# PaddlePaddle/PaddleNLP

Measured on NVIDIA H100. Metric: tokens/sec Llama-3.2-3B seq4096 bf16 pretrain step (global, all GPUs), higher is better.
Workload: dtype bf16

## Files before the change

### paddlenlp_b200/csrc/common.cuh

```cuda
#pragma once
#include <cuda.h>
#include <cuda_bf16.h>
#include <cuda_runtime.h>
#include <stdint.h>
#include <stdio.h>

namespace b200 {

typedef __nv_bfloat16 bf16;

__device__ __forceinline__ uint32_t smem_u32(const void* p) {
  return static_cast<uint32_t>(__cvta_generic_to_shared(p));
}
__device__ __forceinline__ void named_bar_sync(uint32_t id, uint32_t nthreads) {
  asm volatile("bar.sync %0, %1;" ::"r"(id), "r"(nthreads) : "memory");
}

__device__ __forceinline__ void pdl_wait() { asm volatile("griddepcontrol.wait;" ::: "memory"); }
__device__ __forceinline__ void pdl_launch_dependents() { asm volatile("griddepcontrol.launch_dependents;" ::: "memory"); }

__device__ __forceinline__ void mbar_init(uint64_t* bar, uint32_t count) {
  asm volatile("mbarrier.init.shared::cta.b64 [%0], %1;" ::"r"(smem_u32(bar)), "r"(count) : "memory");
}
__device__ __forceinline__ void fence_mbar_init() {
  asm volatile("fence.mbarrier_init.release.cluster;" ::: "memory");
}
__device__ __forceinline__ void fence_proxy_async_smem() {
  asm volatile("fence.proxy.async.shared::cta;" ::: "memory");
}
__device__ __forceinline__ void mbar_arrive_expect_tx(uint64_t* bar, uint32_t bytes) {
  asm volatile("mbarrier.arrive.expect_tx.shared::cta.b64 _, [%0], %1;" ::"r"(smem_u32(bar)), "r"(bytes)
               : "memory");
}
__device__ __forceinline__ void mbar_arrive(uint64_t* bar) {
  asm volatile("mbarrier.arrive.shared::cta.b64 _, [%0];" ::"r"(smem_u32(bar)) : "memory");
}
__device__ __forceinline__ bool mbar_try_wait(uint64_t* bar, uint32_t parity) {
  uint32_t ok;
  asm volatile(
      "{\n\t.reg .pred P;\n\t"
      "mbarrier.try_wait.parity.shared::cta.b64 P, [%1], %2;\n\t"
      "selp.u32 %0, 1, 0, P;\n\t}\n"
      : "=r"(ok)
      : "r"(smem_u32(bar)), "r"(parity)
      : "memory");
  return ok != 0;
}
__device__ __forceinline__ void mbar_wait(uint64_t* bar, uint32_t parity) {
  if (mbar_try_wait(bar, parity)) return;
  long long t0 = clock64();
  uint32_t spins = 0;
  while (!mbar_try_wait(bar, parity)) {
    if ((++spins & 0x3FFu) == 0 && (clock64() - t0) > 8000000000LL) {
      printf("[b200 watchdog] mbarrier wait timed out: block %d thread %d bar 0x%x parity %u\n", (int)blockIdx.x,
             (int)threadIdx.x, smem_u32(bar), parity);
      __trap();
    }
  }
}
__device__ __forceinline__ void mbar_wait_nocall(uint64_t* bar, uint32_t parity) {
  if (mbar_try_wait(bar, parity)) return;
  long long t0 = clock64();
  uint32_t spins = 0;
  while (!mbar_try_wait(bar, parity)) {
    if ((++spins & 0x3FFu) == 0 && (clock64() - t0) > 8000000000LL) __trap();
  }
}

__device__ __forceinline__ void tma_prefetch_desc(const CUtensorMap* tm) {
  asm volatile("prefetch.tensormap [%0];" ::"l"(reinterpret_cast<uint64_t>(tm)) : "memory");
}
__device__ __forceinline__ void tma_load_2d(const CUtensorMap* tm, uint64_t* bar, void* smem_dst, int c0, int c1) {
  asm volatile(
      "cp.async.bulk.tensor.2d.shared::cluster.global.mbarrier::complete_tx::bytes [%0], [%1, {%3, %4}], [%2];"
      ::"r"(smem_u32(smem_dst)), "l"(reinterpret_cast<uint64_t>(tm)), "r"(smem_u32(bar)), "r"(c0), "r"(c1)
      : "memory");
}
__device__ __forceinline__ void bulk_load(void* smem_dst, const void* src, uint32_t bytes, uint64_t* bar) {
  asm volatile("cp.async.bulk.shared::cluster.global.mbarrier::complete_tx::bytes [%0], [%1], %2, [%3];" ::"r"(smem_u32(smem_dst)),
               "l"(src), "r"(bytes), "r"(smem_u32(bar))
               : "memory");
}
__device__ __forceinline__ void tma_load_4d(const CUtensorMap* tm, uint64_t* bar, void* smem_dst, int c0, int c1,
                                            int c2, int c3) {
  asm volatile(
      "cp.async.bulk.tensor.4d.shared::cluster.global.mbarrier::complete_tx::bytes [%0], [%1, {%3, %4, %5, %6}], [%2];"
      ::"r"(smem_u32(smem_dst)), "l"(reinterpret_cast<uint64_t>(tm)), "r"(smem_u32(bar)), "r"(c0), "r"(c1), "r"(c2),
      "r"(c3)
      : "memory");
}
__device__ __forceinline__ void tma_reduce_add_4d(const CUtensorMap* tm, const void* smem_src, int c0, int c1, int c2,
                                                  int c3) {
  asm volatile("cp.reduce.async.bulk.tensor.4d.global.shared::cta.add.tile.bulk_group [%0, {%2, %3, %4, %5}], [%1];" ::"l"(
                   reinterpret_cast<uint64_t>(tm)),
               "r"(smem_u32(smem_src)), "r"(c0), "r"(c1), "r"(c2), "r"(c3)
               : "memory");
}
__device__ __forceinline__ void tma_store_commit() { asm volatile("cp.async.bulk.commit_group;" ::: "memory"); }
template <int N>
__device__ __forceinline__ void tma_store_wait_read() {
  asm volatile("cp.async.bulk.wait_group.read %0;" ::"n"(N) : "memory");
}
template <int N>
__device__ __forceinline__ void tma_store_wait() {
  asm volatile("cp.async.bulk.wait_group %0;" ::"n"(N) : "memory");
}

__device__ __forceinline__ uint64_t wgmma_desc_sw128(uint32_t saddr, uint32_t lbo_bytes, uint32_t sbo_bytes) {
  uint64_t d = 0;
  d |= static_cast<uint64_t>((saddr & 0x3FFFFu) >> 4);
  d |= static_cast<uint64_t>((lbo_bytes >> 4) & 0x3FFFu) << 16;
  d |= static_cast<uint64_t>((sbo_bytes >> 4) & 0x3FFFu) << 32;
  d |= static_cast<uint64_t>(1) << 62;
  return d;
}
__device__ __forceinline__ void wgmma_fence() { asm volatile("wgmma.fence.sync.aligned;" ::: "memory"); }
__device__ __forceinline__ void wgmma_commit() { asm volatile("wgmma.commit_group.sync.aligned;" ::: "memory"); }
template <int N>
__device__ __forceinline__ void wgmma_wait() { asm volatile("wgmma.wait_group.sync.aligned %0;" ::"n"(N) : "memory"); }
template <int R>
__device__ __forceinline__ void setmaxnreg_dec() { asm volatile("setmaxnreg.dec.sync.aligned.u32 %0;" ::"n"(R)); }
template <int R>
__device__ __forceinline__ void setmaxnreg_inc() { asm volatile("setmaxnreg.inc.sync.aligned.u32 %0;" ::"n"(R)); }

template <int TA, int TB>
__device__ __forceinline__ void wgmma_m64n256k16(float (&d)[128], uint64_t desc_a, uint64_t desc_b, uint32_t accumulate) {
  asm volatile(
      "{\n\t.reg .pred p;\n\tsetp.ne.b32 p, %130, 0;\n\t"
      "wgmma.mma_async.sync.aligned.m64n256k16.f32.bf16.bf16 "
      "{%0, %1, %2, %3, %4, %5, %6, %7, %8, %9, %10, %11, %12, %13, %14, %15, %16, %17, %18, %19, %20, %21, %22, %23, %24, %25, %26, %27, %28, %29, %30, %31, %32, %33, %34, %35, %36, %37, %38, %39, %40, %41, %42, %43, %44, %45, %46, %47, %48, %49, %50, %51, %52, %53, %54, %55, %56, %57, %58, %59, %60, %61, %62, %63, %64, %65, %66, %67, %68, %69, %70, %71, %72, %73, %74, %75, %76, %77, %78, %79, %80, %81, %82, %83, %84, %85, %86, %87, %88, %89, %90, %91, %92, %93, %94, %95, %96, %97, %98, %99, %100, %101, %102, %103, %104, %105, %106, %107, %108, %109, %110, %111, %112, %113, %114, %115, %116, %117, %118, %119, %120, %121, %122, %123, %124, %125, %126, %127}, %128, %129, p, 1, 1, %131, %132;\n\t}\n"
      : "+f"(d[0]), "+f"(d[1]), "+f"(d[2]), "+f"(d[3]), "+f"(d[4]), "+f"(d[5]), "+f"(d[6]), "+f"(d[7]), "+f"(d[8]), "+f"(d[9]), "+f"(d[10]), "+f"(d[11]), "+f"(d[12]), "+f"(d[13]), "+f"(d[14]), "+f"(d[15]), "+f"(d[16]), "+f"(d[17]), "+f"(d[18]), "+f"(d[19]), "+f"(d[20]), "+f"(d[21]), "+f"(d[22]), "+f"(d[23]), "+f"(d[24]), "+f"(d[25]), "+f"(d[26]), "+f"(d[27]), "+f"(d[28]), "+f"(d[29]), "+f"(d[30]), "+f"(d[31]), "+f"(d[32]), "+f"(d[33]), "+f"(d[34]), "+f"(d[35]), "+f"(d[36]), "+f"(d[37]), "+f"(d[38]), "+f"(d[39]), "+f"(d[40]), "+f"(d[41]), "+f"(d[42]), "+f"(d[43]), "+f"(d[44]), "+f"(d[45]), "+f"(d[46]), "+f"(d[47]), "+f"(d[48]), "+f"(d[49]), "+f"(d[50]), "+f"(d[51]), "+f"(d[52]), "+f"(d[53]), "+f"(d[54]), "+f"(d[55]), "+f"(d[56]), "+f"(d[57]), "+f"(d[58]), "+f"(d[59]), "+f"(d[60]), "+f"(d[61]), "+f"(d[62]), "+f"(d[63]), "+f"(d[64]), "+f"(d[65]), "+f"(d[66]), "+f"(d[67]), "+f"(d[68]), "+f"(d[69]), "+f"(d[70]), "+f"(d[71]), "+f"(d[72]), "+f"(d[73]), "+f"(d[74]), "+f"(d[75]), "+f"(d[76]), "+f"(d[77]), "+f"(d[78]), "+f"(d[79]), "+f"(d[80]), "+f"(d[81]), "+f"(d[82]), "+f"(d[83]), "+f"(d[84]), "+f"(d[85]), "+f"(d[86]), "+f"(d[87]), "+f"(d[88]), "+f"(d[89]), "+f"(d[90]), "+f"(d[91]), "+f"(d[92]), "+f"(d[93]), "+f"(d[94]), "+f"(d[95]), "+f"(d[96]), "+f"(d[97]), "+f"(d[98]), "+f"(d[99]), "+f"(d[100]), "+f"(d[101]), "+f"(d[102]), "+f"(d[103]), "+f"(d[104]), "+f"(d[105]), "+f"(d[106]), "+f"(d[107]), "+f"(d[108]), "+f"(d[109]), "+f"(d[110]), "+f"(d[111]), "+f"(d[112]), "+f"(d[113]), "+f"(d[114]), "+f"(d[115]), "+f"(d[116]), "+f"(d[117]), "+f"(d[118]), "+f"(d[119]), "+f"(d[120]), "+f"(d[121]), "+f"(d[122]), "+f"(d[123]), "+f"(d[124]), "+f"(d[125]), "+f"(d[126]), "+f"(d[127])
      : "l"(desc_a), "l"(desc_b), "r"(accumulate), "n"(TA), "n"(TB));
}
template <int TA, int TB>
__device__ __forceinline__ void wgmma_m64n64k16(float (&d)[32], uint64_t desc_a, uint64_t desc_b, uint32_t accumulate) {
  asm volatile(
      "{\n\t.reg .pred p;\n\tsetp.ne.b32 p, %34, 0;\n\t"
      "wgmma.mma_async.sync.aligned.m64n64k16.f32.bf16.bf16 "
      "{%0, %1, %2, %3, %4, %5, %6, %7, %8, %9, %10, %11, %12, %13, %14, %15, %16, %17, %18, %19, %20, %21, %22, %23, %24, %25, %26, %27, %28, %29, %30, %31}, %32, %33, p, 1, 1, %35, %36;\n\t}\n"
      : "+f"(d[0]), "+f"(d[1]), "+f"(d[2]), "+f"(d[3]), "+f"(d[4]), "+f"(d[5]), "+f"(d[6]), "+f"(d[7]), "+f"(d[8]), "+f"(d[9]), "+f"(d[10]), "+f"(d[11]), "+f"(d[12]), "+f"(d[13]), "+f"(d[14]), "+f"(d[15]), "+f"(d[16]), "+f"(d[17]), "+f"(d[18]), "+f"(d[19]), "+f"(d[20]), "+f"(d[21]), "+f"(d[22]), "+f"(d[23]), "+f"(d[24]), "+f"(d[25]), "+f"(d[26]), "+f"(d[27]), "+f"(d[28]), "+f"(d[29]), "+f"(d[30]), "+f"(d[31])
      : "l"(desc_a), "l"(desc_b), "r"(accumulate), "n"(TA), "n"(TB));
}
template <int TB>
__device__ __forceinline__ void wgmma_m64n128k16_rs(float (&d)[64], const uint32_t* a, uint64_t desc_b, uint32_t accumulate) {
  asm volatile(
      "{\n\t.reg .pred p;\n\tsetp.ne.b32 p, %69, 0;\n\t"
      "wgmma.mma_async.sync.aligned.m64n128k16.f32.bf16.bf16 "
      "{%0, %1, %2, %3, %4, %5, %6, %7, %8, %9, %10, %11, %12, %13, %14, %15, %16, %17, %18, %19, %20, %21, %22, %23, %24, %25, %26, %27, %28, %29, %30, %31, %32, %33, %34, %35, %36, %37, %38, %39, %40, %41, %42, %43, %44, %45, %46, %47, %48, %49, %50, %51, %52, %53, %54, %55, %56, %57, %58, %59, %60, %61, %62, %63}, {%64, %65, %66, %67}, %68, p, 1, 1, %70;\n\t}\n"
      : "+f"(d[0]), "+f"(d[1]), "+f"(d[2]), "+f"(d[3]), "+f"(d[4]), "+f"(d[5]), "+f"(d[6]), "+f"(d[7]), "+f"(d[8]), "+f"(d[9]), "+f"(d[10]), "+f"(d[11]), "+f"(d[12]), "+f"(d[13]), "+f"(d[14]), "+f"(d[15]), "+f"(d[16]), "+f"(d[17]), "+f"(d[18]), "+f"(d[19]), "+f"(d[20]), "+f"(d[21]), "+f"(d[22]), "+f"(d[23]), "+f"(d[24]), "+f"(d[25]), "+f"(d[26]), "+f"(d[27]), "+f"(d[28]), "+f"(d[29]), "+f"(d[30]), "+f"(d[31]), "+f"(d[32]), "+f"(d[33]), "+f"(d[34]), "+f"(d[35]), "+f"(d[36]), "+f"(d[37]), "+f"(d[38]), "+f"(d[39]), "+f"(d[40]), "+f"(d[41]), "+f"(d[42]), "+f"(d[43]), "+f"(d[44]), "+f"(d[45]), "+f"(d[46]), "+f"(d[47]), "+f"(d[48]), "+f"(d[49]), "+f"(d[50]), "+f"(d[51]), "+f"(d[52]), "+f"(d[53]), "+f"(d[54]), "+f"(d[55]), "+f"(d[56]), "+f"(d[57]), "+f"(d[58]), "+f"(d[59]), "+f"(d[60]), "+f"(d[61]), "+f"(d[62]), "+f"(d[63])
      : "r"(a[0]), "r"(a[1]), "r"(a[2]), "r"(a[3]), "l"(desc_b), "r"(accumulate), "n"(TB));
}
template <int TB>
__device__ __forceinline__ void wgmma_m64n64k16_rs(float (&d)[32], const uint32_t* a, uint64_t desc_b, uint32_t accumulate) {
  asm volatile(
      "{\n\t.reg .pred p;\n\tsetp.ne.b32 p, %37, 0;\n\t"
      "wgmma.mma_async.sync.aligned.m64n64k16.f32.bf16.bf16 "
      "{%0, %1, %2, %3, %4, %5, %6, %7, %8, %9, %10, %11, %12, %13, %14, %15, %16, %17, %18, %19, %20, %21, %22, %23, %24, %25, %26, %27, %28, %29, %30, %31}, {%32, %33, %34, %35}, %36, p, 1, 1, %38;\n\t}\n"
      : "+f"(d[0]), "+f"(d[1]), "+f"(d[2]), "+f"(d[3]), "+f"(d[4]), "+f"(d[5]), "+f"(d[6]), "+f"(d[7]), "+f"(d[8]), "+f"(d[9]), "+f"(d[10]), "+f"(d[11]), "+f"(d[12]), "+f"(d[13]), "+f"(d[14]), "+f"(d[15]), "+f"(d[16]), "+f"(d[17]), "+f"(d[18]), "+f"(d[19]), "+f"(d[20]), "+f"(d[21]), "+f"(d[22]), "+f"(d[23]), "+f"(d[24]), "+f"(d[25]), "+f"(d[26]), "+f"(d[27]), "+f"(d[28]), "+f"(d[29]), "+f"(d[30]), "+f"(d[31])
      : "r"(a[0]), "r"(a[1]), "r"(a[2]), "r"(a[3]), "l"(desc_b), "r"(accumulate), "n"(TB));
}

__device__ __forceinline__ void mma_bf16_16816(float (&c)[4], const uint32_t (&a)[4], uint32_t b0, uint32_t b1) {
  asm volatile(
      "mma.sync.aligned.m16n8k16.row.col.f32.bf16.bf16.f32 {%0, %1, %2, %3}, {%4, %5, %6, %7}, {%8, %9}, "
      "{%0, %1, %2, %3};"
      : "+f"(c[0]), "+f"(c[1]), "+f"(c[2]), "+f"(c[3])
      : "r"(a[0]), "r"(a[1]), "r"(a[2]), "r"(a[3]), "r"(b0), "r"(b1));
}
__device__ __forceinline__ void ldsm_x4(uint32_t saddr, uint32_t (&r)[4]) {
  asm volatile("ldmatrix.sync.aligned.m8n8.x4.shared.b16 {%0, %1, %2, %3}, [%4];"
               : "=r"(r[0]), "=r"(r[1]), "=r"(r[2]), "=r"(r[3])
               : "r"(saddr));
}
__device__ __forceinline__ void ldsm_x4_t(uint32_t saddr, uint32_t (&r)[4]) {
  asm volatile("ldmatrix.sync.aligned.m8n8.x4.trans.shared.b16 {%0, %1, %2, %3}, [%4];"
               : "=r"(r[0]), "=r"(r[1]), "=r"(r[2]), "=r"(r[3])
               : "r"(saddr));
}
__device__ __forceinline__ void cp_async_16(uint32_t saddr, const void* gptr, uint32_t src_bytes) {
  asm volatile("cp.async.cg.shared.global [%0], [%1], 16, %2;" ::"r"(saddr), "l"(gptr), "r"(src_bytes) : "memory");
}
__device__ __forceinline__ void cp_async_commit() { asm volatile("cp.async.commit_group;" ::: "memory"); }
template <int N>
__device__ __forceinline__ void cp_async_wait() { asm volatile("cp.async.wait_group %0;" ::"n"(N) : "memory"); }

__device__ __forceinline__ uint32_t pack_bf16x2(float lo, float hi) {
  __nv_bfloat162 v = __floats2bfloat162_rn(lo, hi);
  return *reinterpret_cast<uint32_t*>(&v);
}
__device__ __forceinline__ float2 unpack_bf16x2(uint32_t u) {
  __nv_bfloat162 v = *reinterpret_cast<__nv_bfloat162*>(&u);
  return __bfloat1622float2(v);
}
__device__ __forceinline__ float bf16_round(float x) { return __bfloat162float(__float2bfloat16_rn(x)); }

__device__ __forceinline__ uint4 ld_nc_v4(const void* p) {
  uint4 r;
  asm("ld.global.nc.L1::no_allocate.v4.u32 {%0, %1, %2, %3}, [%4];"
               : "=r"(r.x), "=r"(r.y), "=r"(r.z), "=r"(r.w)
               : "l"(p));
  return r;
}
__device__ __forceinline__ void st_na_v4(void* p, const uint4& v) {
  asm volatile("st.global.L1::no_allocate.v4.u32 [%0], {%1, %2, %3, %4};" ::"l"(p), "r"(v.x), "r"(v.y), "r"(v.z),
               "r"(v.w));
}
__device__ __forceinline__ uint4 ld_shared_v4(uint32_t saddr) {
  uint4 r;
  asm volatile("ld.shared.v4.u32 {%0, %1, %2, %3}, [%4];" : "=r"(r.x), "=r"(r.y), "=r"(r.z), "=r"(r.w) : "r"(saddr));
  return r;
}

__device__ __forceinline__ float fast_exp2(float x) {
  float y;
  asm("ex2.approx.ftz.f32 %0, %1;" : "=f"(y) : "f"(x));
  return y;
}
__device__ __forceinline__ float fast_rcp(float x) {
  float y;
  asm("rcp.approx.ftz.f32 %0, %1;" : "=f"(y) : "f"(x));
  return y;
}

struct f32x2 { float x, y; };
__device__ __forceinline__ f32x2 f2_mul(f32x2 a, f32x2 b) { return f32x2{__fmul_rn(a.x, b.x), __fmul_rn(a.y, b.y)}; }
__device__ __forceinline__ f32x2 f2_add(f32x2 a, f32x2 b) { return f32x2{__fadd_rn(a.x, b.x), __fadd_rn(a.y, b.y)}; }
__device__ __forceinline__ f32x2 f2_fma(f32x2 a, f32x2 b, f32x2 c) {
  return f32x2{__fmaf_rn(a.x, b.x, c.x), __fmaf_rn(a.y, b.y, c.y)};
}

__device__ __forceinline__ uint32_t swiglu_fwd_pair(uint32_t g2, uint32_t u2) {
  const float2 gf = unpack_bf16x2(g2), uf = unpack_bf16x2(u2);
  const f32x2 g{gf.x, gf.y}, u{uf.x, uf.y}, one{1.f, 1.f};
  const f32x2 t = f2_mul(g, f32x2{-1.4426950408889634f, -1.4426950408889634f});
  const f32x2 a = f2_add(f32x2{fast_exp2(t.x), fast_exp2(t.y)}, one);
  const f32x2 sg{fast_rcp(a.x), fast_rcp(a.y)};
  const f32x2 m = f2_mul(f2_mul(g, sg), u);
  return pack_bf16x2(m.x, m.y);
}

__device__ __forceinline__ void swiglu_bwd_pair(uint32_t g2, uint32_t u2, float d0, float d1, uint32_t& dg2, uint32_t& du2) {
  const float2 gf = unpack_bf16x2(g2), uf = unpack_bf16x2(u2);
  const f32x2 g{gf.x, gf.y}, u{uf.x, uf.y}, d{d0, d1}, one{1.f, 1.f};
  const f32x2 t = f2_mul(g, f32x2{-1.4426950408889634f, -1.4426950408889634f});
  const f32x2 a = f2_add(f32x2{fast_exp2(t.x), fast_exp2(t.y)}, one);
  const f32x2 sg{fast_rcp(a.x), fast_rcp(a.y)};
  const f32x2 silu = f2_mul(g, sg);
  const f32x2 om = f2_fma(sg, f32x2{-1.f, -1.f}, one);
  const f32x2 ds = f2_mul(sg, f2_fma(g, om, one));
  const f32x2 dgv = f2_mul(f2_mul(d, u), ds);
  const f32x2 duv = f2_mul(d, silu);
  dg2 = pack_bf16x2(dgv.x, dgv.y);
  du2 = pack_bf16x2(duv.x, duv.y);
}

__device__ __forceinline__ float warp_sum(float v) {
#pragma unroll
  for (int o = 16; o > 0; o >>= 1) v += __shfl_xor_sync(0xffffffffu, v, o);
  return v;
}

constexpr int DECODE_PART_ROW = 132;
constexpr int DECODE_PART_M = 128;

}
```

### paddlenlp_b200/csrc/gemm_wgmma.cu

```cuda
#include "../../include/b200nlp.h"
#include <cstdlib>
#include <cstring>

#include "common.cuh"
#include "host_util.h"

namespace b200 {
namespace gemm {

constexpr int BN = 256;
constexpr int BK = 64;
constexpr int B_BYTES = BN * BK * 2;

template <int NWG>
struct Tile {
  static constexpr int BM = 64 * NWG;
  static constexpr int NUM_THREADS = 128 * (NWG + 1);
  static constexpr int A_BYTES = BM * BK * 2;
  static constexpr int STAGE_BYTES = A_BYTES + B_BYTES;
  static constexpr int STAGES = NWG == 2 ? 4 : 5;
  static constexpr int SMEM_BYTES = STAGES * STAGE_BYTES + 256 + 1024;
};
static int tile_wgs(int64_t M) { return M <= 64 ? 1 : 2; }

struct Params {
  int M, N, K;
  int num_m_tiles, num_n_tiles;
  int epi_mode;
  int swiglu_inter;
  int gm;
  int split_k;
  int kb_per_split;
  const float* bias;
  bf16* c;
  int64_t ldc;
  const bf16* r;
  int64_t ldr;
  bf16* aux;
  int64_t ld_aux;
  float* ws;
};

__device__ __forceinline__ void tile_coords(int t, int num_m, int num_n, int& m_blk, int& n_blk, int GM) {
  const int per_group = GM * num_n;
  const int g = t / per_group;
  const int first_m = g * GM;
  const int gsize = min(GM, num_m - first_m);
  const int r = t - g * per_group;
  m_blk = first_m + (r % gsize);
  n_blk = r / gsize;
}

__device__ __forceinline__ void fence_acc(float (&acc)[128]) {
#pragma unroll
  for (int i = 0; i < 128; ++i) asm volatile("" : "+f"(acc[i])::"memory");
}

__device__ __forceinline__ void store_bf16x2(bf16* base, int64_t ld, int row, int col, int N, float v0, float v1) {
  bf16* dst = base + static_cast<int64_t>(row) * ld + col;
  if (col + 1 < N) *reinterpret_cast<uint32_t*>(dst) = pack_bf16x2(v0, v1);
  else if (col < N) *dst = __float2bfloat16_rn(v0);
}

template <int NWG, bool A_MN, bool B_MN>
__global__ void __launch_bounds__(Tile<NWG>::NUM_THREADS, 1)
gemm_bf16_kernel(const __grid_constant__ CUtensorMap tmA, const __grid_constant__ CUtensorMap tmB, const Params p) {
  using T = Tile<NWG>;
  constexpr int BM = T::BM, A_BYTES = T::A_BYTES, STAGE_BYTES = T::STAGE_BYTES, STAGES = T::STAGES;
  extern __shared__ uint8_t smem_raw[];
  uint8_t* smem = reinterpret_cast<uint8_t*>((reinterpret_cast<uintptr_t>(smem_raw) + 1023) & ~uintptr_t(1023));
  uint64_t* full_bar = reinterpret_cast<uint64_t*>(smem + STAGES * STAGE_BYTES);
  uint64_t* empty_bar = full_bar + STAGES;

  const int num_items = p.num_m_tiles * p.num_n_tiles * p.split_k;
  const int num_kb_total = (p.K + BK - 1) / BK;
  if (threadIdx.x == 0) {
    tma_prefetch_desc(&tmA);
    tma_prefetch_desc(&tmB);
    for (int i = 0; i < STAGES; ++i) {
      mbar_init(&full_bar[i], 1);
      mbar_init(&empty_bar[i], NWG * 128);
    }
    fence_mbar_init();
  }
  __syncthreads();
  pdl_launch_dependents();
  pdl_wait();

  const int wg = threadIdx.x >> 7;
  if (wg == 0) {
    setmaxnreg_dec<40>();
    if (threadIdx.x == 0) {
      uint32_t it = 0;
      for (int t = blockIdx.x; t < num_items; t += gridDim.x) {
        int m_blk, n_blk;
        tile_coords(t / p.split_k, p.num_m_tiles, p.num_n_tiles, m_blk, n_blk, p.gm);
        const int kb0 = (t % p.split_k) * p.kb_per_split;
        const int kb1 = min(num_kb_total, kb0 + p.kb_per_split);
        for (int kb = kb0; kb < kb1; ++kb, ++it) {
          const int st = static_cast<int>(it % STAGES);
          mbar_wait(&empty_bar[st], ((it / STAGES) & 1u) ^ 1u);
          uint8_t* sA = smem + st * STAGE_BYTES;
          uint8_t* sB = sA + A_BYTES;
          mbar_arrive_expect_tx(&full_bar[st], STAGE_BYTES);
          if constexpr (A_MN) {
#pragma unroll
            for (int h = 0; h < NWG; ++h) tma_load_2d(&tmA, &full_bar[st], sA + h * (64 * BK * 2), m_blk * BM + 64 * h, kb * BK);
          } else {
            tma_load_2d(&tmA, &full_bar[st], sA, kb * BK, m_blk * BM);
          }
          if constexpr (B_MN) {
#pragma unroll
            for (int h = 0; h < 4; ++h) {
              const int c0 = p.epi_mode == 4 ? (h >> 1) * p.swiglu_inter + n_blk * 128 + (h & 1) * 64 : n_blk * BN + h * 64;
              tma_load_2d(&tmB, &full_bar[st], sB + h * (B_BYTES / 4), c0, kb * BK);
            }
          } else {
            tma_load_2d(&tmB, &full_bar[st], sB, kb * BK, n_blk * BN);
            tma_load_2d(&tmB, &full_bar[st], sB + B_BYTES / 2, kb * BK, n_blk * BN + 128);
          }
        }
      }
    }
    return;
  }

  setmaxnreg_inc<232>();
  const int cw = wg - 1;
  const int wi = (threadIdx.x >> 5) & 3, lane = threadIdx.x & 31;
  const uint32_t ring = smem_u32(smem);
  constexpr uint32_t A_KSTEP = A_MN ? 2048u : 32u, B_KSTEP = B_MN ? 2048u : 32u;
  const uint32_t a_off = static_cast<uint32_t>(cw) * (64 * BK * 2);
  uint32_t it = 0;
  float acc[128];
  for (int t = blockIdx.x; t < num_items; t += gridDim.x) {
    int m_blk, n_blk;
    tile_coords(t / p.split_k, p.num_m_tiles, p.num_n_tiles, m_blk, n_blk, p.gm);
    const int kb0 = (t % p.split_k) * p.kb_per_split;
    const int nkb = min(num_kb_total, kb0 + p.kb_per_split) - kb0;
    fence_acc(acc);
#pragma unroll
    for (int i = 0; i < 128; ++i) acc[i] = 0.f;
    fence_acc(acc);
    for (int i = 0; i < nkb; ++i, ++it) {
      const int st = static_cast<int>(it % STAGES);
      mbar_wait(&full_bar[st], (it / STAGES) & 1u);
      const uint32_t sA = ring + st * STAGE_BYTES + a_off, sB = ring + st * STAGE_BYTES + A_BYTES;
      const uint64_t dA = wgmma_desc_sw128(sA, A_MN ? 64 * BK * 2 : 16, 1024);
      const uint64_t dB = wgmma_desc_sw128(sB, B_MN ? B_BYTES / 4 : 16, 1024);
      wgmma_fence();
#pragma unroll
      for (int kk = 0; kk < BK / 16; ++kk)
        wgmma_m64n256k16<A_MN ? 1 : 0, B_MN ? 1 : 0>(acc, dA + ((kk * A_KSTEP) >> 4), dB + ((kk * B_KSTEP) >> 4),
                                                     (i > 0 || kk > 0) ? 1u : 0u);
      wgmma_commit();
      wgmma_wait<1>();
      if (i > 0) mbar_arrive(&empty_bar[(it - 1) % STAGES]);
    }
    wgmma_wait<0>();
    fence_acc(acc);
    if (nkb > 0) mbar_arrive(&empty_bar[(it - 1) % STAGES]);

    const int row_base = m_blk * BM + cw * 64 + wi * 16 + (lane >> 2);
    const int cq = 2 * (lane & 3);
    if (p.epi_mode == 4) {
#pragma unroll
      for (int i = 0; i < 2; ++i) {
        const int row = row_base + 8 * i;
        if (row >= p.M) continue;
#pragma unroll
        for (int j = 0; j < 16; ++j) {
          const int ch = n_blk * 128 + 8 * j + cq;
          if (ch >= p.swiglu_inter) continue;
          const uint32_t gp = pack_bf16x2(acc[4 * j + 2 * i], acc[4 * j + 2 * i + 1]);
          const uint32_t up = pack_bf16x2(acc[4 * (j + 16) + 2 * i], acc[4 * (j + 16) + 2 * i + 1]);
          if (p.aux != nullptr) {
            bf16* g = p.aux + static_cast<int64_t>(row) * p.ld_aux + ch;
            *reinterpret_cast<uint32_t*>(g) = gp;
            *reinterpret_cast<uint32_t*>(g + p.swiglu_inter) = up;
          }
          *reinterpret_cast<uint32_t*>(p.c + static_cast<int64_t>(row) * p.ldc + ch) = swiglu_fwd_pair(gp, up);
        }
      }
      continue;
    }
    if (p.epi_mode == 5) {
#pragma unroll
      for (int i = 0; i < 2; ++i) {
        const int row = row_base + 8 * i;
        if (row >= p.M) continue;
        const bf16* gu = p.aux + static_cast<int64_t>(row) * p.ld_aux;
        bf16* dgu = p.c + static_cast<int64_t>(row) * p.ldc;
#pragma unroll
        for (int j = 0; j < 32; ++j) {
          const int ch = n_blk * BN + 8 * j + cq;
          if (ch >= p.N) continue;
          const float2 dr = unpack_bf16x2(pack_bf16x2(acc[4 * j + 2 * i], acc[4 * j + 2 * i + 1]));
          uint32_t dg2, du2;
          swiglu_bwd_pair(*reinterpret_cast<const uint32_t*>(gu + ch), *reinterpret_cast<const uint32_t*>(gu + p.swiglu_inter + ch),
                          dr.x, dr.y, dg2, du2);
          *reinterpret_cast<uint32_t*>(dgu + ch) = dg2;
          *reinterpret_cast<uint32_t*>(dgu + p.swiglu_inter + ch) = du2;
        }
      }
      continue;
    }
#pragma unroll
    for (int i = 0; i < 2; ++i) {
      const int row = row_base + 8 * i;
      if (row >= p.M) continue;
#pragma unroll
      for (int j = 0; j < 32; ++j) {
        const int col = n_blk * BN + 8 * j + cq;
        if (col >= p.N) continue;
        float f0 = acc[4 * j + 2 * i], f1 = acc[4 * j + 2 * i + 1];
        if (p.epi_mode == 3) {
          float* w = p.ws + static_cast<int64_t>(row) * p.N + col;
          asm volatile("red.global.add.v2.f32 [%0], {%1, %2};" ::"l"(w), "f"(f0), "f"(f1) : "memory");
          continue;
        }
        if (p.bias != nullptr) {
          f0 += __ldg(p.bias + col);
          if (col + 1 < p.N) f1 += __ldg(p.bias + col + 1);
        }
        if (p.epi_mode == 1 || p.epi_mode == 2) {
          const bf16* o = p.epi_mode == 1 ? p.c + static_cast<int64_t>(row) * p.ldc + col : p.r + static_cast<int64_t>(row) * p.ldr + col;
          if (p.epi_mode == 2) { f0 = bf16_round(f0); f1 = bf16_round(f1); }
          f0 += __bfloat162float(o[0]);
          if (col + 1 < p.N) f1 += __bfloat162float(o[1]);
        }
        store_bf16x2(p.c, p.ldc, row, col, p.N, f0, f1);
      }
    }
  }
}

template <int NWG, bool A_MN, bool B_MN>
static int launch(const CUtensorMap& tmA, const CUtensorMap& tmB, const Params& p, int max_ctas, cudaStream_t stream) {
  using T = Tile<NWG>;
  constexpr int SMEM_BYTES = T::SMEM_BYTES;
  auto kern = gemm_bf16_kernel<NWG, A_MN, B_MN>;
  static bool attr_set = false;
  if (!attr_set) {
    cudaError_t e = cudaFuncSetAttribute(kern, cudaFuncAttributeMaxDynamicSharedMemorySize, SMEM_BYTES);
    if (e != cudaSuccess) {
      set_last_error("cudaFuncSetAttribute(gemm smem=%d): %s", SMEM_BYTES, cudaGetErrorString(e));
      return static_cast<int>(e);
    }
    attr_set = true;
  }
  const int num_items = p.num_m_tiles * p.num_n_tiles * p.split_k;
  int ctas = sm_count();
  if (max_ctas > 0 && max_ctas < ctas) ctas = max_ctas;
  if (ctas > num_items) ctas = num_items;
  Params pp = p;
  pp.gm = (16ll * 128 * p.K * 2 <= (18ll << 20)) ? 16 : 8;
  cudaError_t e = launch_pdl(kern, dim3(ctas), dim3(T::NUM_THREADS), SMEM_BYTES, stream, tmA, tmB, pp);
  if (e != cudaSuccess) {
    set_last_error("gemm launch: %s", cudaGetErrorString(e));
    return static_cast<int>(e);
  }
  return 0;
}

static int dispatch(bool a_mn, bool b_mn, const CUtensorMap& tmA, const CUtensorMap& tmB, const Params& p, int max_ctas,
                    cudaStream_t stream) {
  if (tile_wgs(p.M) == 1) {
    if (a_mn && b_mn) return launch<1, true, true>(tmA, tmB, p, max_ctas, stream);
    if (a_mn) return launch<1, true, false>(tmA, tmB, p, max_ctas, stream);
    if (b_mn) return launch<1, false, true>(tmA, tmB, p, max_ctas, stream);
    return launch<1, false, false>(tmA, tmB, p, max_ctas, stream);
  }
  if (a_mn && b_mn) return launch<2, true, true>(tmA, tmB, p, max_ctas, stream);
  if (a_mn) return launch<2, true, false>(tmA, tmB, p, max_ctas, stream);
  if (b_mn) return launch<2, false, true>(tmA, tmB, p, max_ctas, stream);
  return launch<2, false, false>(tmA, tmB, p, max_ctas, stream);
}

static int make_a_map(CUtensorMap* tm, const void* A, int64_t M, int64_t K, int64_t lda, bool mn) {
  uint64_t dims[2], strides[1] = {static_cast<uint64_t>(lda) * 2};
  uint32_t box[2];
  if (mn) { dims[0] = M; dims[1] = K; box[0] = 64; box[1] = BK; }
  else    { dims[0] = K; dims[1] = M; box[0] = BK; box[1] = 64 * tile_wgs(M); }
  return encode_tmap_bf16(tm, A, 2, dims, strides, box);
}
static int make_b_map(CUtensorMap* tm, const void* B, int64_t N, int64_t K, int64_t ldb, bool mn) {
  uint64_t dims[2], strides[1] = {static_cast<uint64_t>(ldb) * 2};
  uint32_t box[2];
  if (mn) { dims[0] = N; dims[1] = K; box[0] = 64; box[1] = BK; }
  else    { dims[0] = K; dims[1] = N; box[0] = BK; box[1] = 128; }
  return encode_tmap_bf16(tm, B, 2, dims, strides, box);
}

static Params base_params(int64_t M, int64_t N, int64_t K) {
  Params p = {};
  p.M = static_cast<int>(M);
  p.N = static_cast<int>(N);
  p.K = static_cast<int>(K);
  const int64_t bm = 64 * tile_wgs(M);
  p.num_m_tiles = static_cast<int>((M + bm - 1) / bm);
  p.num_n_tiles = static_cast<int>((N + BN - 1) / BN);
  p.split_k = 1;
  p.kb_per_split = static_cast<int>((K + BK - 1) / BK);
  return p;
}

}
}

extern "C" int b200_gemm_bf16_ex(const void* A, const void* B, void* C, const float* bias, const void* residual,
                                 int64_t M, int64_t N, int64_t K, int64_t lda, int64_t ldb, int64_t ldc, int64_t ldr,
                                 int a_mn_major, int b_mn_major, int accumulate, int max_ctas, cudaStream_t stream) {
  using namespace b200;
  using namespace b200::gemm;
  B200_CHECK_ARG(A && B && C, "gemm: null pointer");
  B200_CHECK_ARG(M > 0 && N > 0 && K > 0, "gemm: non-positive dimension M=%lld N=%lld K=%lld", (long long)M,
                 (long long)N, (long long)K);
  B200_CHECK_ARG(lda % 8 == 0 && ldb % 8 == 0 && ldc % 8 == 0, "gemm: leading dimensions must be multiples of 8");
  B200_CHECK_ARG(!(residual && accumulate), "gemm: residual and accumulate are mutually exclusive");
  B200_CHECK_ARG(!residual || ldr % 8 == 0, "gemm: ldr must be a multiple of 8");
  B200_CHECK_ARG(M < (1ll << 31) && N < (1ll << 31) && K < (1ll << 31), "gemm: dimension too large");
  CUtensorMap tmA, tmB;
  int rc;
  if ((rc = make_a_map(&tmA, A, M, K, lda, a_mn_major)) != 0) return rc;
  if ((rc = make_b_map(&tmB, B, N, K, ldb, b_mn_major)) != 0) return rc;
  Params p = base_params(M, N, K);
  p.epi_mode = residual ? 2 : (accumulate ? 1 : 0);
  p.bias = bias;
  p.c = static_cast<bf16*>(C);
  p.ldc = ldc;
  p.r = static_cast<const bf16*>(residual);
  p.ldr = ldr;
  return dispatch(a_mn_major, b_mn_major, tmA, tmB, p, max_ctas, stream);
}

extern "C" int b200_gemm_swiglu_bf16(const void* X, const void* W, void* GU, void* Mout, int64_t M, int64_t inter, int64_t K,
                                     int64_t ldx, int64_t ldw, int64_t ldgu, int64_t ldm, cudaStream_t stream) {
  using namespace b200;
  using namespace b200::gemm;
  B200_CHECK_ARG(X && W && Mout, "gemm_swiglu: null pointer");
  B200_CHECK_ARG(M > 0 && inter > 0 && K > 0 && inter % 64 == 0, "gemm_swiglu: intermediate size must be a multiple of 64 (got %lld)",
                 (long long)inter);
  B200_CHECK_ARG(ldx % 8 == 0 && ldw % 8 == 0 && ldgu % 8 == 0 && ldm % 8 == 0, "gemm_swiglu: leading dimensions must be multiples of 8");
  B200_CHECK_ARG(M < (1ll << 31) && inter < (1ll << 30) && K < (1ll << 31), "gemm_swiglu: dimension too large");
  CUtensorMap tmA, tmB;
  int rc;
  if ((rc = make_a_map(&tmA, X, M, K, ldx, false)) != 0) return rc;
  if ((rc = make_b_map(&tmB, W, 2 * inter, K, ldw, true)) != 0) return rc;
  Params p = base_params(M, 2 * inter, K);
  p.num_n_tiles = static_cast<int>((inter + 127) / 128);
  p.epi_mode = 4;
  p.swiglu_inter = static_cast<int>(inter);
  p.c = static_cast<bf16*>(Mout);
  p.ldc = ldm;
  p.aux = static_cast<bf16*>(GU);
  p.ld_aux = ldgu;
  return dispatch(false, true, tmA, tmB, p, 0, stream);
}

extern "C" int b200_gemm_swiglu_bwd_bf16(const void* dY, const void* Wdown, const void* GU, void* DGU, int64_t M, int64_t inter,
                                         int64_t K, int64_t lddy, int64_t ldw, int64_t ldgu, int64_t lddgu, cudaStream_t stream) {
  using namespace b200;
  using namespace b200::gemm;
  B200_CHECK_ARG(dY && Wdown && GU && DGU, "gemm_swiglu_bwd: null pointer");
  B200_CHECK_ARG(M > 0 && inter > 0 && K > 0 && inter % 64 == 0, "gemm_swiglu_bwd: intermediate size must be a multiple of 64 (got %lld)",
                 (long long)inter);
  B200_CHECK_ARG(lddy % 8 == 0 && ldw % 8 == 0 && ldgu % 8 == 0 && lddgu % 8 == 0, "gemm_swiglu_bwd: leading dimensions must be multiples of 8");
  B200_CHECK_ARG(M < (1ll << 31) && inter < (1ll << 30) && K < (1ll << 31), "gemm_swiglu_bwd: dimension too large");
  CUtensorMap tmA, tmB;
  int rc;
  if ((rc = make_a_map(&tmA, dY, M, K, lddy, false)) != 0) return rc;
  if ((rc = make_b_map(&tmB, Wdown, inter, K, ldw, false)) != 0) return rc;
  Params p = base_params(M, inter, K);
  p.epi_mode = 5;
  p.swiglu_inter = static_cast<int>(inter);
  p.c = static_cast<bf16*>(DGU);
  p.ldc = lddgu;
  p.aux = const_cast<bf16*>(static_cast<const bf16*>(GU));
  p.ld_aux = ldgu;
  return dispatch(false, false, tmA, tmB, p, 0, stream);
}

namespace b200 {
namespace gemm {
__global__ void splitk_finish_kernel(float* __restrict__ ws, const float* __restrict__ bias, bf16* __restrict__ out,
                                     int64_t M, int64_t N, int64_t ldc) {
  const int64_t nch = N >> 3;
  const int64_t total = M * nch;
  for (int64_t i = blockIdx.x * static_cast<int64_t>(blockDim.x) + threadIdx.x; i < total;
       i += static_cast<int64_t>(gridDim.x) * blockDim.x) {
    const int64_t r = i / nch, c = i % nch;
    float4* src = reinterpret_cast<float4*>(ws + r * N) + 2 * c;
    float4 a = src[0], b = src[1];
    src[0] = make_float4(0.f, 0.f, 0.f, 0.f);
    src[1] = make_float4(0.f, 0.f, 0.f, 0.f);
    if (bias != nullptr) {
      const float4* bp = reinterpret_cast<const float4*>(bias) + 2 * c;
      const float4 b0 = __ldg(bp), b1 = __ldg(bp + 1);
      a.x += b0.x; a.y += b0.y; a.z += b0.z; a.w += b0.w;
      b.x += b1.x; b.y += b1.y; b.z += b1.z; b.w += b1.w;
    }
    uint4 o;
    o.x = pack_bf16x2(a.x, a.y); o.y = pack_bf16x2(a.z, a.w);
    o.z = pack_bf16x2(b.x, b.y); o.w = pack_bf16x2(b.z, b.w);
    *(reinterpret_cast<uint4*>(out + r * ldc) + c) = o;
  }
}
}
}

extern "C" int64_t b200_gemm_splitk_workspace_bytes(int64_t M, int64_t N) { return M * N * 4; }

extern "C" int b200_gemm_bf16_splitk(const void* A, const void* B, void* C, const float* bias, void* workspace, int64_t M,
                                     int64_t N, int64_t K, int64_t lda, int64_t ldb, int64_t ldc, int a_mn_major,
                                     int b_mn_major, int split_k, cudaStream_t stream) {
  using namespace b200;
  using namespace b200::gemm;
  B200_CHECK_ARG(A && B && workspace, "gemm_splitk: null pointer");
  B200_CHECK_ARG(M > 0 && N > 0 && K > 0 && N % 8 == 0, "gemm_splitk: bad dimensions (N must be a multiple of 8)");
  B200_CHECK_ARG(lda % 8 == 0 && ldb % 8 == 0 && ldc % 8 == 0, "gemm_splitk: leading dimensions must be multiples of 8");
  CUtensorMap tmA, tmB;
  int rc;
  if ((rc = make_a_map(&tmA, A, M, K, lda, a_mn_major)) != 0) return rc;
  if ((rc = make_b_map(&tmB, B, N, K, ldb, b_mn_major)) != 0) return rc;
  Params p = base_params(M, N, K);
  const int num_kb = p.kb_per_split;
  const int tiles = p.num_m_tiles * p.num_n_tiles;
  if (split_k <= 0) {
    const int sms = sm_count();
    split_k = (sms + tiles - 1) / tiles;
    if (split_k > num_kb / 4) split_k = num_kb / 4;
    if (split_k < 1) split_k = 1;
  }
  p.kb_per_split = (num_kb + split_k - 1) / split_k;
  p.split_k = (num_kb + p.kb_per_split - 1) / p.kb_per_split;
  p.epi_mode = 3;
  p.ws = static_cast<float*>(workspace);
  if ((rc = dispatch(a_mn_major, b_mn_major, tmA, tmB, p, 0, stream)) != 0) return rc;
  if (C == nullptr) return 0;
  const int64_t total = M * (N / 8);
  int64_t blocks = (total + 255) / 256;
  if (blocks > sm_count() * 8) blocks = sm_count() * 8;
  splitk_finish_kernel<<<static_cast<unsigned>(blocks), 256, 0, stream>>>(static_cast<float*>(workspace), bias,
                                                                         static_cast<bf16*>(C), M, N, ldc);
  return check_launch("gemm_splitk(finish)");
}

extern "C" int b200_gemm_bf16(const void* A, const void* B, void* C, const float* bias, int64_t M, int64_t N, int64_t K,
                              int64_t lda, int64_t ldb, int64_t ldc, int a_mn_major, int b_mn_major, int accumulate,
                              cudaStream_t stream) {
  return b200_gemm_bf16_ex(A, B, C, bias, nullptr, M, N, K, lda, ldb, ldc, 0, a_mn_major, b_mn_major, accumulate,
                           0, stream);
}
```

Baseline: 19900.

## Stage GEMM epilogue through swizzled shared memory and store tiles with TMA

```diff
diff --git a/paddlenlp_b200/csrc/common.cuh b/paddlenlp_b200/csrc/common.cuh
--- a/paddlenlp_b200/csrc/common.cuh
+++ b/paddlenlp_b200/csrc/common.cuh
@@ -96,6 +96,16 @@
                "r"(smem_u32(smem_src)), "r"(c0), "r"(c1), "r"(c2), "r"(c3)
                : "memory");
 }
+__device__ __forceinline__ void tma_store_2d(const CUtensorMap* tm, uint32_t smem_src, int c0, int c1) {
+  asm volatile("cp.async.bulk.tensor.2d.global.shared::cta.bulk_group [%0, {%2, %3}], [%1];" ::"l"(reinterpret_cast<uint64_t>(tm)),
+               "r"(smem_src), "r"(c0), "r"(c1)
+               : "memory");
+}
+__device__ __forceinline__ void tma_prefetch_l2_2d(const CUtensorMap* tm, int c0, int c1) {
+  asm volatile("cp.async.bulk.prefetch.tensor.2d.L2.global.tile [%0, {%1, %2}];" ::"l"(reinterpret_cast<uint64_t>(tm)), "r"(c0),
+               "r"(c1)
+               : "memory");
+}
 __device__ __forceinline__ void tma_store_commit() { asm volatile("cp.async.bulk.commit_group;" ::: "memory"); }
 template <int N>
 __device__ __forceinline__ void tma_store_wait_read() {
@@ -204,6 +214,9 @@
 __device__ __forceinline__ void st_na_v4(void* p, const uint4& v) {
   asm volatile("st.global.L1::no_allocate.v4.u32 [%0], {%1, %2, %3, %4};" ::"l"(p), "r"(v.x), "r"(v.y), "r"(v.z),
                "r"(v.w));
+}
+__device__ __forceinline__ void st_shared_u32(uint32_t saddr, uint32_t v) {
+  asm volatile("st.shared.u32 [%0], %1;" ::"r"(saddr), "r"(v));
 }
 __device__ __forceinline__ uint4 ld_shared_v4(uint32_t saddr) {
   uint4 r;
diff --git a/paddlenlp_b200/csrc/gemm_wgmma.cu b/paddlenlp_b200/csrc/gemm_wgmma.cu
--- a/paddlenlp_b200/csrc/gemm_wgmma.cu
+++ b/paddlenlp_b200/csrc/gemm_wgmma.cu
@@ -11,6 +11,8 @@
 constexpr int BN = 256;
 constexpr int BK = 64;
 constexpr int B_BYTES = BN * BK * 2;
+constexpr int EPI_BOX = 64;
+constexpr int EPI_BOX_BYTES = EPI_BOX * EPI_BOX * 2;
 
 template <int NWG>
 struct Tile {
@@ -19,7 +21,8 @@
   static constexpr int A_BYTES = BM * BK * 2;
   static constexpr int STAGE_BYTES = A_BYTES + B_BYTES;
   static constexpr int STAGES = NWG == 2 ? 4 : 5;
-  static constexpr int SMEM_BYTES = STAGES * STAGE_BYTES + 256 + 1024;
+  static constexpr int EPI_BYTES = NWG == 2 ? NWG * 2 * EPI_BOX_BYTES : 0;
+  static constexpr int SMEM_BYTES = STAGES * STAGE_BYTES + EPI_BYTES + 256 + 1024;
 };
 static int tile_wgs(int64_t M) { return M <= 64 ? 1 : 2; }
 
@@ -39,6 +42,7 @@
   bf16* aux;
   int64_t ld_aux;
   float* ws;
+  int smem_epi;
 };
 
 __device__ __forceinline__ void tile_coords(int t, int num_m, int num_n, int& m_blk, int& n_blk, int GM) {
@@ -62,14 +66,48 @@
   else if (col < N) *dst = __float2bfloat16_rn(v0);
 }
 
+__device__ __forceinline__ uint32_t epi_slot(uint32_t buf, int r, int jj, int lane) {
+  return buf + r * 128 + ((jj ^ (r & 7)) << 4) + 4 * (lane & 3);
+}
+template <int KEEP>
+__device__ __forceinline__ void epi_begin(int cw, bool leader) {
+  if (leader) tma_store_wait_read<KEEP>();
+  named_bar_sync(1 + cw, 128);
+}
+__device__ __forceinline__ void epi_end(int cw) {
+  fence_proxy_async_smem();
+  named_bar_sync(1 + cw, 128);
+}
+__device__ __forceinline__ uint32_t ld_pair(const bf16* base, int64_t ld, int row, int col, int M, int N) {
+  if (row >= M || col >= N) return 0u;
+  const bf16* src = base + static_cast<int64_t>(row) * ld + col;
+  if (col + 1 < N) return *reinterpret_cast<const uint32_t*>(src);
+  return static_cast<uint32_t>(__bfloat16_as_ushort(*src));
+}
+__device__ __forceinline__ void epi_prefetch(const CUtensorMap* tmC, const CUtensorMap* tmX, const Params& p, int n_blk, int row0) {
+  for (int s = 0; s < BN / EPI_BOX; ++s) {
+    const int col0 = n_blk * BN + EPI_BOX * s;
+    if (col0 >= p.N) break;
+    if (p.epi_mode == 1) {
+      tma_prefetch_l2_2d(tmC, col0, row0);
+    } else if (p.epi_mode == 2) {
+      tma_prefetch_l2_2d(tmX, col0, row0);
+    } else {
+      tma_prefetch_l2_2d(tmX, col0, row0);
+      tma_prefetch_l2_2d(tmX, p.swiglu_inter + col0, row0);
+    }
+  }
+}
+
 template <int NWG, bool A_MN, bool B_MN>
 __global__ void __launch_bounds__(Tile<NWG>::NUM_THREADS, 1)
-gemm_bf16_kernel(const __grid_constant__ CUtensorMap tmA, const __grid_constant__ CUtensorMap tmB, const Params p) {
+gemm_bf16_kernel(const __grid_constant__ CUtensorMap tmA, const __grid_constant__ CUtensorMap tmB,
+                 const __grid_constant__ CUtensorMap tmC, const __grid_constant__ CUtensorMap tmX, const Params p) {
   using T = Tile<NWG>;
   constexpr int BM = T::BM, A_BYTES = T::A_BYTES, STAGE_BYTES = T::STAGE_BYTES, STAGES = T::STAGES;
   extern __shared__ uint8_t smem_raw[];
   uint8_t* smem = reinterpret_cast<uint8_t*>((reinterpret_cast<uintptr_t>(smem_raw) + 1023) & ~uintptr_t(1023));
-  uint64_t* full_bar = reinterpret_cast<uint64_t*>(smem + STAGES * STAGE_BYTES);
+  uint64_t* full_bar = reinterpret_cast<uint64_t*>(smem + STAGES * STAGE_BYTES + T::EPI_BYTES);
   uint64_t* empty_bar = full_bar + STAGES;
 
   const int num_items = p.num_m_tiles * p.num_n_tiles * p.split_k;
@@ -131,6 +169,10 @@
   const uint32_t ring = smem_u32(smem);
   constexpr uint32_t A_KSTEP = A_MN ? 2048u : 32u, B_KSTEP = B_MN ? 2048u : 32u;
   const uint32_t a_off = static_cast<uint32_t>(cw) * (64 * BK * 2);
+  const bool leader = (threadIdx.x & 127) == 0;
+  const bool prefetch = p.smem_epi && leader && (p.epi_mode == 1 || p.epi_mode == 2 || p.epi_mode == 5);
+  const uint32_t ebuf = smem_u32(smem + STAGES * STAGE_BYTES) + cw * 2 * EPI_BOX_BYTES;
+  uint32_t nbox = 0;
   uint32_t it = 0;
   float acc[128];
   for (int t = blockIdx.x; t < num_items; t += gridDim.x) {
@@ -138,6 +180,7 @@
     tile_coords(t / p.split_k, p.num_m_tiles, p.num_n_tiles, m_blk, n_blk, p.gm);
     const int kb0 = (t % p.split_k) * p.kb_per_split;
     const int nkb = min(num_kb_total, kb0 + p.kb_per_split) - kb0;
+    const int prefetch_kb = nkb > 8 ? nkb - 8 : 0;
     fence_acc(acc);
 #pragma unroll
     for (int i = 0; i < 128; ++i) acc[i] = 0.f;
@@ -154,6 +197,9 @@
         wgmma_m64n256k16<A_MN ? 1 : 0, B_MN ? 1 : 0>(acc, dA + ((kk * A_KSTEP) >> 4), dB + ((kk * B_KSTEP) >> 4),
                                                      (i > 0 || kk > 0) ? 1u : 0u);
       wgmma_commit();
+      if constexpr (NWG == 2) {
+        if (prefetch && i == prefetch_kb) epi_prefetch(&tmC, &tmX, p, n_blk, m_blk * BM + cw * 64);
+      }
       wgmma_wait<1>();
       if (i > 0) mbar_arrive(&empty_bar[(it - 1) % STAGES]);
     }
@@ -163,6 +209,126 @@
 
     const int row_base = m_blk * BM + cw * 64 + wi * 16 + (lane >> 2);
     const int cq = 2 * (lane & 3);
+    if constexpr (NWG == 2) {
+      if (p.smem_epi) {
+        const int row0 = m_blk * BM + cw * 64;
+        const int r_lo = wi * 16 + (lane >> 2);
+        if (p.epi_mode == 4) {
+#pragma unroll
+          for (int h = 0; h < 2; ++h) {
+            const int ch0 = n_blk * 128 + EPI_BOX * h;
+            if (ch0 >= p.swiglu_inter) continue;
+            if (p.aux != nullptr) {
+              epi_begin<0>(cw, leader);
+#pragma unroll
+              for (int i = 0; i < 2; ++i)
+#pragma unroll
+                for (int jj = 0; jj < 8; ++jj) {
+                  const int j = 8 * h + jj;
+                  st_shared_u32(epi_slot(ebuf, r_lo + 8 * i, jj, lane), pack_bf16x2(acc[4 * j + 2 * i], acc[4 * j + 2 * i + 1]));
+                  st_shared_u32(epi_slot(ebuf + EPI_BOX_BYTES, r_lo + 8 * i, jj, lane),
+                                pack_bf16x2(acc[4 * (j + 16) + 2 * i], acc[4 * (j + 16) + 2 * i + 1]));
+                }
+              epi_end(cw);
+              if (leader) {
+                tma_store_2d(&tmX, ebuf, ch0, row0);
+                tma_store_2d(&tmX, ebuf + EPI_BOX_BYTES, p.swiglu_inter + ch0, row0);
+                tma_store_commit();
+              }
+            }
+            epi_begin<0>(cw, leader);
+#pragma unroll
+            for (int i = 0; i < 2; ++i)
+#pragma unroll
+              for (int jj = 0; jj < 8; ++jj) {
+                const int j = 8 * h + jj;
+                const uint32_t gp = pack_bf16x2(acc[4 * j + 2 * i], acc[4 * j + 2 * i + 1]);
+                const uint32_t up = pack_bf16x2(acc[4 * (j + 16) + 2 * i], acc[4 * (j + 16) + 2 * i + 1]);
+                st_shared_u32(epi_slot(ebuf, r_lo + 8 * i, jj, lane), swiglu_fwd_pair(gp, up));
+              }
+            epi_end(cw);
+            if (leader) {
+              tma_store_2d(&tmC, ebuf, ch0, row0);
+              tma_store_commit();
+            }
+          }
+          continue;
+        }
+        if (p.epi_mode == 5) {
+#pragma unroll
+          for (int s = 0; s < BN / EPI_BOX; ++s) {
+            const int ch0 = n_blk * BN + EPI_BOX * s;
+            if (ch0 >= p.N) continue;
+            epi_begin<0>(cw, leader);
+#pragma unroll
+            for (int q = 0; q < 4; ++q) {
+              const int i = q >> 1, jj0 = 4 * (q & 1);
+              uint32_t g[4], u[4];
+#pragma unroll
+              for (int k = 0; k < 4; ++k) {
+                const int row = row0 + r_lo + 8 * i, ch = ch0 + 8 * (jj0 + k) + cq;
+                g[k] = ld_pair(p.aux, p.ld_aux, row, ch, p.M, p.N);
+                u[k] = ld_pair(p.aux + p.swiglu_inter, p.ld_aux, row, ch, p.M, p.N);
+              }
+#pragma unroll
+              for (int k = 0; k < 4; ++k) {
+                const int jj = jj0 + k, j = 8 * s + jj;
+                uint32_t dg2, du2;
+                swiglu_bwd_pair(g[k], u[k], bf16_round(acc[4 * j + 2 * i]), bf16_round(acc[4 * j + 2 * i + 1]), dg2, du2);
+                st_shared_u32(epi_slot(ebuf, r_lo + 8 * i, jj, lane), dg2);
+                st_shared_u32(epi_slot(ebuf + EPI_BOX_BYTES, r_lo + 8 * i, jj, lane), du2);
+              }
+            }
+            epi_end(cw);
+            if (leader) {
+              tma_store_2d(&tmC, ebuf, ch0, row0);
+              tma_store_2d(&tmC, ebuf + EPI_BOX_BYTES, p.swiglu_inter + ch0, row0);
+              tma_store_commit();
+            }
+          }
+          continue;
+        }
+#pragma unroll
+        for (int s = 0; s < BN / EPI_BOX; ++s) {
+          const int col0 = n_blk * BN + EPI_BOX * s;
+          if (col0 >= p.N) continue;
+          const uint32_t buf = ebuf + (nbox++ & 1u) * EPI_BOX_BYTES;
+          epi_begin<1>(cw, leader);
+#pragma unroll
+          for (int i = 0; i < 2; ++i) {
+            uint32_t o[8];
+            if (p.epi_mode != 0) {
+              const bf16* src = p.epi_mode == 1 ? p.c : p.r;
+              const int64_t ld = p.epi_mode == 1 ? p.ldc : p.ldr;
+#pragma unroll
+              for (int jj = 0; jj < 8; ++jj) o[jj] = ld_pair(src, ld, row0 + r_lo + 8 * i, col0 + 8 * jj + cq, p.M, p.N);
+            }
+#pragma unroll
+            for (int jj = 0; jj < 8; ++jj) {
+              const int j = 8 * s + jj, col = col0 + 8 * jj + cq;
+              float f0 = acc[4 * j + 2 * i], f1 = acc[4 * j + 2 * i + 1];
+              if (p.bias != nullptr) {
+                if (col < p.N) f0 += __ldg(p.bias + col);
+                if (col + 1 < p.N) f1 += __ldg(p.bias + col + 1);
+              }
+              if (p.epi_mode != 0) {
+                if (p.epi_mode == 2) { f0 = bf16_round(f0); f1 = bf16_round(f1); }
+                const float2 of = unpack_bf16x2(o[jj]);
+                f0 += of.x;
+                f1 += of.y;
+              }
+              st_shared_u32(epi_slot(buf, r_lo + 8 * i, jj, lane), pack_bf16x2(f0, f1));
+            }
+          }
+          epi_end(cw);
+          if (leader) {
+            tma_store_2d(&tmC, buf, col0, row0);
+            tma_store_commit();
+          }
+        }
+        continue;
+      }
+    }
     if (p.epi_mode == 4) {
 #pragma unroll
       for (int i = 0; i < 2; ++i) {
@@ -233,10 +399,14 @@
       }
     }
   }
+  if constexpr (NWG == 2) {
+    if (leader) tma_store_wait<0>();
+  }
 }
 
 template <int NWG, bool A_MN, bool B_MN>
-static int launch(const CUtensorMap& tmA, const CUtensorMap& tmB, const Params& p, int max_ctas, cudaStream_t stream) {
+static int launch(const CUtensorMap& tmA, const CUtensorMap& tmB, const CUtensorMap& tmC, const CUtensorMap& tmX, const Params& p,
+                  int max_ctas, cudaStream_t stream) {
   using T = Tile<NWG>;
   constexpr int SMEM_BYTES = T::SMEM_BYTES;
   auto kern = gemm_bf16_kernel<NWG, A_MN, B_MN>;
@@ -255,7 +425,7 @@
   if (ctas > num_items) ctas = num_items;
   Params pp = p;
   pp.gm = (16ll * 128 * p.K * 2 <= (18ll << 20)) ? 16 : 8;
-  cudaError_t e = launch_pdl(kern, dim3(ctas), dim3(T::NUM_THREADS), SMEM_BYTES, stream, tmA, tmB, pp);
+  cudaError_t e = launch_pdl(kern, dim3(ctas), dim3(T::NUM_THREADS), SMEM_BYTES, stream, tmA, tmB, tmC, tmX, pp);
   if (e != cudaSuccess) {
     set_last_error("gemm launch: %s", cudaGetErrorString(e));
     return static_cast<int>(e);
@@ -263,18 +433,57 @@
   return 0;
 }
 
-static int dispatch(bool a_mn, bool b_mn, const CUtensorMap& tmA, const CUtensorMap& tmB, const Params& p, int max_ctas,
+static int make_epi_map(CUtensorMap* tm, const void* base, int64_t rows, int64_t cols, int64_t ld) {
+  const uint64_t dims[2] = {static_cast<uint64_t>(cols), static_cast<uint64_t>(rows)}, strides[1] = {static_cast<uint64_t>(ld) * 2};
+  const uint32_t box[2] = {EPI_BOX, EPI_BOX};
+  return encode_tmap_bf16(tm, base, 2, dims, strides, box);
+}
+static bool aligned16(const void* ptr) { return (reinterpret_cast<uintptr_t>(ptr) & 15) == 0; }
+
+static int setup_smem_epilogue(Params& p, CUtensorMap* tmC, CUtensorMap* tmX) {
+  p.smem_epi = 0;
+  if (tile_wgs(p.M) != 2 || p.epi_mode == 3 || !aligned16(p.c)) return 0;
+  int rc = 0;
+  switch (p.epi_mode) {
+    case 2:
+      if (!aligned16(p.r)) return 0;
+      if ((rc = make_epi_map(tmX, p.r, p.M, p.N, p.ldr)) != 0) return rc;
+      rc = make_epi_map(tmC, p.c, p.M, p.N, p.ldc);
+      break;
+    case 4:
+      if (p.aux != nullptr && !aligned16(p.aux)) return 0;
+      if (p.aux != nullptr && (rc = make_epi_map(tmX, p.aux, p.M, p.N, p.ld_aux)) != 0) return rc;
+      rc = make_epi_map(tmC, p.c, p.M, p.swiglu_inter, p.ldc);
+      break;
+    case 5:
+      if (!aligned16(p.aux)) return 0;
+      if ((rc = make_epi_map(tmX, p.aux, p.M, 2ll * p.N, p.ld_aux)) != 0) return rc;
+      rc = make_epi_map(tmC, p.c, p.M, 2ll * p.N, p.ldc);
+      break;
+    default:
+      rc = make_epi_map(tmC, p.c, p.M, p.N, p.ldc);
+  }
+  if (rc == 0) p.smem_epi = 1;
+  return rc;
+}
+
+static int dispatch(bool a_mn, bool b_mn, const CUtensorMap& tmA, const CUtensorMap& tmB, Params p, int max_ctas,
                     cudaStream_t stream) {
+  CUtensorMap tmC, tmX;
+  memset(&tmC, 0, sizeof(tmC));
+  memset(&tmX, 0, sizeof(tmX));
+  int rc;
+  if ((rc = setup_smem_epilogue(p, &tmC, &tmX)) != 0) return rc;
   if (tile_wgs(p.M) == 1) {
-    if (a_mn && b_mn) return launch<1, true, true>(tmA, tmB, p, max_ctas, stream);
-    if (a_mn) return launch<1, true, false>(tmA, tmB, p, max_ctas, stream);
-    if (b_mn) return launch<1, false, true>(tmA, tmB, p, max_ctas, stream);
-    return launch<1, false, false>(tmA, tmB, p, max_ctas, stream);
-  }
-  if (a_mn && b_mn) return launch<2, true, true>(tmA, tmB, p, max_ctas, stream);
-  if (a_mn) return launch<2, true, false>(tmA, tmB, p, max_ctas, stream);
-  if (b_mn) return launch<2, false, true>(tmA, tmB, p, max_ctas, stream);
-  return launch<2, false, false>(tmA, tmB, p, max_ctas, stream);
+    if (a_mn && b_mn) return launch<1, true, true>(tmA, tmB, tmC, tmX, p, max_ctas, stream);
+    if (a_mn) return launch<1, true, false>(tmA, tmB, tmC, tmX, p, max_ctas, stream);
+    if (b_mn) return launch<1, false, true>(tmA, tmB, tmC, tmX, p, max_ctas, stream);
+    return launch<1, false, false>(tmA, tmB, tmC, tmX, p, max_ctas, stream);
+  }
+  if (a_mn && b_mn) return launch<2, true, true>(tmA, tmB, tmC, tmX, p, max_ctas, stream);
+  if (a_mn) return launch<2, true, false>(tmA, tmB, tmC, tmX, p, max_ctas, stream);
+  if (b_mn) return launch<2, false, true>(tmA, tmB, tmC, tmX, p, max_ctas, stream);
+  return launch<2, false, false>(tmA, tmB, tmC, tmX, p, max_ctas, stream);
 }
 
 static int make_a_map(CUtensorMap* tm, const void* A, int64_t M, int64_t K, int64_t lda, bool mn) {
```

Result: faster. 21630 (median of 6 runs) (+8.7%).
